# plumk97/pip

Measured on AMD Instinct MI355X. Metric: GiB/s payload checksummed (device-resident), MTU-9000 TCP batch; Mpkt/s, higher is better.
Workload: dtype u8

## Files before the change

### pip_amd/csrc/pipck_coop.hip

```cpp
#include "pipck_common.hpp"
#include "pipck_device.hpp"

#include <algorithm>

namespace pipck {

constexpr uint32_t kCoopLoadsOnly = 1u << 21;
constexpr uint32_t kCoopNoEnd = 1u << 22;

template <int U>
constexpr int coop_waves_per_simd() { return U >= 32 ? 2 : (U >= 24 ? 3 : (U >= 16 ? 4 : 5)); }

__host__ __device__ constexpr uint32_t coop_pitch(uint32_t k) { return k | 1u; }

template <int U, bool VERIFY, bool NT, bool PROBE>
__device__ __forceinline__ void coop_body(uint32_t* s_part, const uint8_t* __restrict__ arena, uint32_t cpp,
                                          uint32_t len, uint64_t n, uint32_t K, const uint32_t* __restrict__ pseudo,
                                          uint32_t n_flows, const uint32_t* __restrict__ flow_of, uint64_t flow_origin,
                                          uint16_t* __restrict__ out, uint8_t* __restrict__ ok, uint32_t kflags,
                                          uint32_t* __restrict__ err) {
    if (!PROBE) kflags &= ~(kCoopLoadsOnly | kCoopNoEnd);
    const int lane = threadIdx.x & 63;
    const uint32_t w = (uint32_t)__builtin_amdgcn_readfirstlane((int)(threadIdx.x >> 6));
    const uint32_t pitch = coop_pitch(K);
    const uint64_t p0 = (uint64_t)blockIdx.x * K;
    const uint32_t np = (uint32_t)min<uint64_t>((uint64_t)K, n - p0);
    const uint32_t tchunks = np * cpp;
    const uint32_t rows = (tchunks + 63) >> 6;
    const uint32_t nch = (len + 15) >> 4;
    const int tail = nch ? (int)len - 16 * ((int)nch - 1) : 16;
    for (uint32_t i = threadIdx.x; i < 64u * pitch; i += 256) s_part[i] = 0;
    uint32_t Pb = 0;
    bool fbad = false;
    if (pseudo && threadIdx.x < np) {
        const uint64_t pkt = p0 + threadIdx.x;
        Pb = flow_of ? flow_pseudo(pseudo, flow_of[pkt], n_flows, fbad)
                     : pseudo[(uint32_t)((flow_origin + pkt) % n_flows)];
    }
    __syncthreads();
    const buf_t tb = buf_rsrc(reinterpret_cast<const u32x4*>(arena) + p0 * cpp, tchunks * 16u);
    uint32_t* part = s_part + lane * pitch;
    const uint32_t q = 256u / cpp, rm = 256u % cpp;
    uint32_t pkt = (64u * w) / cpp, k0 = (64u * w) % cpp;
    const uint32_t my_rows = rows > w ? (rows - w + 3) >> 2 : 0u;
    u32x4 v[U];
    uint32_t probe = 0;
#pragma unroll
    for (int u = 0; u < U; u++) v[u] = buf_load<NT>(tb, ((w + 4u * u) * 64u + lane) * 16u);
    for (uint32_t j0 = 0; j0 < my_rows; j0 += U) {
#pragma unroll
        for (int u = 0; u < U; u++) {
            const uint32_t j = j0 + u;
            if (j < my_rows && (kflags & kCoopLoadsOnly)) {
                probe += v[u].x;
            } else if (j < my_rows) {
                uint32_t k = k0 + lane, pk = pkt;
                if (k >= cpp) {
                    k -= cpp;
                    pk++;
                }
                u32x4 x = v[u];
                if (k >= nch) x = u32x4{0u, 0u, 0u, 0u};
                else if (k == nch - 1 && tail < 16) x = mask_tail(x, tail);
                if (pk < np) atomicAdd(&part[pk], dot4(x, 0u));
                k0 += rm;
                pkt += q;
                if (k0 >= cpp) {
                    k0 -= cpp;
                    pkt++;
                }
            }
            v[u] = buf_load<NT>(tb, ((w + 4u * (j + U)) * 64u + lane) * 16u);
        }
    }
    __syncthreads();
    if (kflags & (kCoopLoadsOnly | kCoopNoEnd)) {
        if (probe == 0x9E3779B9u) s_part[0] = probe;
        return;
    }
    const uint32_t i = threadIdx.x;
    if (i < np) {
        uint32_t s = 0;
#pragma unroll 16
        for (int l = 0; l < 64; l++) s += s_part[l * pitch + i];
        const uint32_t F = bswap16(fold16(s));
        const uint32_t P = pseudo ? Pb + len_term(len) : 0u;
        if (fbad) flow_refused(err);
        if (VERIFY)
            store_result8(buf_rsrc(ok + p0, np), i, fbad ? 0u : (uint32_t)(fold16(P + F) == 0xFFFFu));
        else
            store_result16(buf_rsrc(out + p0, 2u * np), 2u * i, fbad ? 0u : (uint32_t)finish(P, F));
    }
}

template <int U, bool VERIFY, bool NT>
__global__ __launch_bounds__(256) __attribute__((amdgpu_waves_per_eu(coop_waves_per_simd<U>()))) void k_flat_coop(
    const uint8_t* __restrict__ arena, uint32_t cpp, uint32_t len, uint64_t n, uint32_t K,
    const uint32_t* __restrict__ pseudo, uint32_t n_flows, const uint32_t* __restrict__ flow_of, uint64_t flow_origin,
    uint16_t* __restrict__ out, uint8_t* __restrict__ ok, uint32_t kflags, uint32_t* __restrict__ err) {
    extern __shared__ uint32_t s_part[];
    coop_body<U, VERIFY, NT, false>(s_part, arena, cpp, len, n, K, pseudo, n_flows, flow_of, flow_origin, out, ok,
                                    kflags, err);
}

template <int U, bool VERIFY, bool NT>
__global__ __launch_bounds__(256) __attribute__((amdgpu_waves_per_eu(coop_waves_per_simd<U>()))) void
k_flat_coop_probe(const uint8_t* __restrict__ arena, uint32_t cpp, uint32_t len, uint64_t n, uint32_t K,
                  const uint32_t* __restrict__ pseudo, uint32_t n_flows, const uint32_t* __restrict__ flow_of,
                  uint64_t flow_origin, uint16_t* __restrict__ out, uint8_t* __restrict__ ok, uint32_t kflags,
                  uint32_t* __restrict__ err) {
    extern __shared__ uint32_t s_part[];
    coop_body<U, VERIFY, NT, true>(s_part, arena, cpp, len, n, K, pseudo, n_flows, flow_of, flow_origin, out, ok,
                                   kflags, err);
}

typedef void (*coop_fn)(const uint8_t*, uint32_t, uint32_t, uint64_t, uint32_t, const uint32_t*, uint32_t,
                        const uint32_t*, uint64_t, uint16_t*, uint8_t*, uint32_t, uint32_t*);

int launch_flat_coop(bool verify, const void* d_arena, uint64_t stride, uint32_t len, uint64_t n,
                     const uint32_t* d_pseudo, uint32_t n_flows, const uint32_t* d_flow_of, uint64_t flow_origin,
                     uint16_t* d_out, uint8_t* d_ok, uint32_t* d_err, hipStream_t s, uint32_t rows_per_wave,
                     uint32_t ring, uint32_t kflags) {
    const uint32_t cpp = (uint32_t)(stride / 16);
    const bool jumbo = cpp >= 256;
    const uint32_t rpw = rows_per_wave ? rows_per_wave : (jumbo ? 64u : 48u);
    uint32_t K = (4u * rpw * 64u) / cpp;
    K = std::max<uint32_t>(8u, std::min<uint32_t>(256u, K / 8u * 8u));
    if ((uint64_t)K * cpp * 16u >= (1ull << 31)) return PIPCK_EINVAL;
    const uint64_t blocks = (n + K - 1) / K;
    if (blocks > 0x7FFFFFFFull) return PIPCK_EINVAL;
    const size_t lds = 64u * coop_pitch(K) * sizeof(uint32_t);
    const uint32_t nf = n_flows ? n_flows : 1u;
    const uint32_t u = ring ? ring : 32u;
    static const coop_fn kCoop[3][2] = {
        {k_flat_coop<16, false, true>, k_flat_coop<16, true, true>},
        {k_flat_coop<24, false, true>, k_flat_coop<24, true, true>},
        {k_flat_coop<32, false, true>, k_flat_coop<32, true, true>}};
    static const coop_fn kCoopProbe[3] = {k_flat_coop_probe<16, false, true>, k_flat_coop_probe<24, false, true>,
                                          k_flat_coop_probe<32, false, true>};
    const int ui = u >= 32 ? 2 : (u >= 24 ? 1 : 0);
    const bool probe = (kflags & (kCoopLoadsOnly | kCoopNoEnd)) && !verify;
    PIPCK_LAUNCH(probe ? kCoopProbe[ui] : kCoop[ui][verify], dim3((uint32_t)blocks), dim3(256), lds, s, (const uint8_t*)d_arena, cpp, len, n,
                 K, d_pseudo, nf, d_flow_of, flow_origin, d_out, d_ok, kflags, d_err);
    PIPCK_LAUNCHED("k_flat_coop");
    return PIPCK_OK;
}

}
```

### pip_amd/engine.py

```python
from __future__ import annotations

import ctypes as C

from . import _lib
from ._lib import Desc, Flow4, Flow6, call, check, load

DESC_BYTES = C.sizeof(Desc)


def _torch():
    import torch

    return torch


def _ptr(t) -> C.c_void_p | None:
    return None if t is None else C.c_void_p(t.data_ptr())


def current_stream(device=None) -> C.c_void_p:
    torch = _torch()
    return C.c_void_p(torch.cuda.current_stream(device).cuda_stream)


def require_gpu() -> None:
    torch = _torch()
    if not torch.cuda.is_available():
        raise RuntimeError("pip_amd engine needs a HIP device (gfx950); none is visible")
    load()


_hip = None


def hip_runtime() -> C.CDLL:
    global _hip
    if _hip is None:
        import os

        load()
        paths = set()
        with open("/proc/self/maps") as f:
            for line in f:
                parts = line.split()
                if len(parts) >= 6 and os.path.basename(parts[5]).startswith("libamdhip64.so"):
                    paths.add(os.path.realpath(parts[5]))
        if len(paths) != 1:
            raise RuntimeError(f"expected exactly one HIP runtime mapped in this process, found {sorted(paths)}")
        _hip = C.CDLL(paths.pop(), mode=os.RTLD_NOLOAD | os.RTLD_GLOBAL)
    return _hip


def pci_bus_id(device: int) -> str:
    buf = C.create_string_buffer(64)
    try:
        if hip_runtime().hipDeviceGetPCIBusId(buf, C.c_int(len(buf)), C.c_int(device)) == 0:
            return buf.value.decode()
    except (OSError, RuntimeError):
        pass
    p = _torch().cuda.get_device_properties(device)
    return f"{getattr(p, 'pci_domain_id', 0):04x}:{getattr(p, 'pci_bus_id', 0):02x}:" \
           f"{getattr(p, 'pci_device_id', 0):02x}.0"


def gen_flows(family: int, n_flows: int, seed: int, proto: int, device=None):
    torch = _torch()
    size = C.sizeof(Flow4 if family == 4 else Flow6)
    flows = torch.empty(n_flows * size, dtype=torch.uint8, device=device or "cuda")
    fn = "pipck_gen_flows4" if family == 4 else "pipck_gen_flows6"
    call(fn, _ptr(flows), n_flows, seed, proto, current_stream(flows.device))
    return flows, prepare_flows(family, flows, n_flows)


def prepare_flows(family: int, flows, n_flows: int):
    torch = _torch()
    pseudo = torch.empty(n_flows, dtype=torch.int32, device=flows.device)
    fn = "pipck_flows4_prepare" if family == 4 else "pipck_flows6_prepare"
    call(fn, _ptr(flows), n_flows, _ptr(pseudo), current_stream(flows.device))
    return pseudo


def flows_to_device(family: int, flows_bytes: bytes, device=None):
    torch = _torch()
    t = torch.frombuffer(bytearray(flows_bytes), dtype=torch.uint8).to(device or "cuda")
    return t


def _n_flows(n_flows, pseudo, flow_of) -> int:
    if n_flows is not None:
        return n_flows
    if flow_of is not None and pseudo is not None:
        return pseudo.numel()
    return 1


def checksum_fixed(arena, stride: int, length: int, n: int, pseudo=None, n_flows: int | None = None, flow_of=None,
                   flow_origin: int = 0, out=None, err=None):
    torch = _torch()
    if out is None:
        out = torch.empty(n, dtype=torch.int16, device=arena.device)
    _check_span(arena, stride, length, n)
    call("pipck_checksum_fixed_n", _ptr(arena), stride, length, n, _ptr(pseudo), _n_flows(n_flows, pseudo, flow_of),
         _ptr(flow_of), flow_origin, _ptr(out), _ptr(err), current_stream(arena.device))
    return out


def _bound(fn: str, *args):
    f = getattr(load(), fn)

    def run():
        rc = f(*args)
        if rc:
            check(fn, rc)

    return run


def prepare_checksum_fixed(arena, stride: int, length: int, n: int, pseudo=None, n_flows: int | None = None,
                           flow_of=None, flow_origin: int = 0, out=None, err=None):
    torch = _torch()
    if out is None:
        out = torch.empty(n, dtype=torch.int16, device=arena.device)
    _check_span(arena, stride, length, n)
    return _bound("pipck_checksum_fixed_n", _ptr(arena), stride, length, n, _ptr(pseudo),
                  _n_flows(n_flows, pseudo, flow_of), _ptr(flow_of), flow_origin, _ptr(out), _ptr(err),
                  current_stream(arena.device)), out


def verify_fixed(arena, stride: int, length: int, n: int, pseudo=None, n_flows: int | None = None, flow_of=None,
                 flow_origin: int = 0, ok=None, err=None):
    torch = _torch()
    if ok is None:
        ok = torch.empty(n, dtype=torch.uint8, device=arena.device)
    _check_span(arena, stride, length, n)
    call("pipck_verify_fixed_n", _ptr(arena), stride, length, n, _ptr(pseudo), _n_flows(n_flows, pseudo, flow_of),
         _ptr(flow_of), flow_origin, _ptr(ok), _ptr(err), current_stream(arena.device))
    return ok


def checksum_ragged(arena, desc, pseudo=None, out=None, err=None):
    torch = _torch()
    n = desc.shape[0]
    if out is None:
        out = torch.empty(n, dtype=torch.int16, device=arena.device)
    call("pipck_checksum_ragged_n", _ptr(arena), _nbytes(arena), _ptr(desc), n, _ptr(pseudo),
         pseudo.numel() if pseudo is not None else 0, _ptr(out), _ptr(err), current_stream(arena.device))
    return out


def verify_ragged(arena, desc, pseudo=None, ok=None, err=None):
    torch = _torch()
    n = desc.shape[0]
    if ok is None:
        ok = torch.empty(n, dtype=torch.uint8, device=arena.device)
    call("pipck_verify_ragged_n", _ptr(arena), _nbytes(arena), _ptr(desc), n, _ptr(pseudo),
         pseudo.numel() if pseudo is not None else 0, _ptr(ok), _ptr(err), current_stream(arena.device))
    return ok


def tune_xcd_weights(m=None, period: int = 0) -> None:
    arr = (C.c_uint32 * 8)(*[int(x) for x in m]) if m is not None else None
    call("pipck_tune_xcd_weights", arr, period)


def _nbytes(t) -> int:
    return t.numel() * t.element_size()


def checksum_packed(arena, lens, tile_chunk, n: int | None = None, pseudo=None, n_flows: int | None = None,
                    flow_of=None, flow_origin: int = 0, out=None, err=None):
    torch = _torch()
    n = lens.numel() if n is None else n
    if out is None:
        out = torch.empty(n, dtype=torch.int16, device=arena.device)
    _check_packed(arena, lens, tile_chunk, n)
    call("pipck_checksum_packed_n", _ptr(arena), _nbytes(arena), _ptr(lens), _ptr(tile_chunk), n, _ptr(pseudo),
         _n_flows(n_flows, pseudo, flow_of), _ptr(flow_of), flow_origin, _ptr(out), _ptr(err),
         current_stream(arena.device))
    return out


def verify_packed(arena, lens, tile_chunk, n: int | None = None, pseudo=None, n_flows: int | None = None,
                  flow_of=None, flow_origin: int = 0, ok=None, err=None):
    torch = _torch()
    n = lens.numel() if n is None else n
    if ok is None:
        ok = torch.empty(n, dtype=torch.uint8, device=arena.device)
    _check_packed(arena, lens, tile_chunk, n)
    call("pipck_verify_packed_n", _ptr(arena), _nbytes(arena), _ptr(lens), _ptr(tile_chunk), n, _ptr(pseudo),
         _n_flows(n_flows, pseudo, flow_of), _ptr(flow_of), flow_origin, _ptr(ok), _ptr(err),
         current_stream(arena.device))
    return ok


def packed_index(lens, n: int | None = None):
    torch = _torch()
    n = lens.numel() if n is None else n
    tc = torch.empty((n + 63) // 64 + 1, dtype=torch.int64, device=lens.device)
    call("pipck_packed_index", _ptr(lens), n, _ptr(tc), current_stream(lens.device))
    return tc


_packed_total: dict = {}


def _check_packed(arena, lens, tile_chunk, n, unit: int = 16):
    import weakref

    if n > lens.numel() or tile_chunk.numel() < (n + 63) // 64 + 1:
        raise ValueError("lens / tile_chunk shorter than the batch")
    ent = _packed_total.get(id(tile_chunk))
    if ent is not None and ent[0]() is tile_chunk and ent[1] == tile_chunk._version and ent[2] == n:
        chunks = ent[3]
    else:
        chunks = int(tile_chunk[(n + 63) // 64].item())
        if len(_packed_total) > 64:
            _packed_total.clear()
        _packed_total[id(tile_chunk)] = (weakref.ref(tile_chunk), tile_chunk._version, n, chunks)
    need = unit * chunks if unit == 16 else (chunks + 15) // 16 * 16
    if need > arena.numel() * arena.element_size():
        raise ValueError(f"packed batch needs {need} B, arena has {arena.numel() * arena.element_size()}")


def checksum_packed_bytes(arena, lens, tile_off, n: int | None = None, pseudo=None, n_flows: int | None = None,
                          flow_of=None, flow_origin: int = 0, out=None, err=None):
    torch = _torch()
    n = lens.numel() if n is None else n
    if out is None:
        out = torch.empty(n, dtype=torch.int16, device=arena.device)
    _check_packed(arena, lens, tile_off, n, unit=1)
    call("pipck_checksum_packed_bytes_n", _ptr(arena), _nbytes(arena), _ptr(lens), _ptr(tile_off), n, _ptr(pseudo),
         _n_flows(n_flows, pseudo, flow_of), _ptr(flow_of), flow_origin, _ptr(out), _ptr(err),
         current_stream(arena.device))
    return out


def prepare_checksum_packed_bytes(arena, lens, tile_off, n: int | None = None, pseudo=None,
                                  n_flows: int | None = None, flow_of=None, flow_origin: int = 0, out=None, err=None):
    torch = _torch()
    n = lens.numel() if n is None else n
    if out is None:
        out = torch.empty(n, dtype=torch.int16, device=arena.device)
    _check_packed(arena, lens, tile_off, n, unit=1)
    return _bound("pipck_checksum_packed_bytes_n", _ptr(arena), _nbytes(arena), _ptr(lens), _ptr(tile_off), n,
                  _ptr(pseudo), _n_flows(n_flows, pseudo, flow_of), _ptr(flow_of), flow_origin, _ptr(out),
                  _ptr(err), current_stream(arena.device)), out


def verify_packed_bytes(arena, lens, tile_off, n: int | None = None, pseudo=None, n_flows: int | None = None,
                        flow_of=None, flow_origin: int = 0, ok=None, err=None):
    torch = _torch()
    n = lens.numel() if n is None else n
    if ok is None:
        ok = torch.empty(n, dtype=torch.uint8, device=arena.device)
    _check_packed(arena, lens, tile_off, n, unit=1)
    call("pipck_verify_packed_bytes_n", _ptr(arena), _nbytes(arena), _ptr(lens), _ptr(tile_off), n, _ptr(pseudo),
         _n_flows(n_flows, pseudo, flow_of), _ptr(flow_of), flow_origin, _ptr(ok), _ptr(err),
         current_stream(arena.device))
    return ok


def rx_verify_ring(ring, stride: int, lens, n: int | None = None, ok=None, err=None):
    torch = _torch()
    n = lens.numel() if n is None else n
    if n * stride > _nbytes(ring) or n > lens.numel():
        raise ValueError("ring smaller than n * stride, or fewer lengths than slots")
    if ok is None:
        ok = torch.empty(n, dtype=torch.uint8, device=ring.device)
    call("pipck_rx_verify_ring_n", _ptr(ring), stride, _ptr(lens), n, _ptr(ok), _ptr(err),
         current_stream(ring.device))
    return ok


def rx_verify_device(arena, lens, tile_off, n: int | None = None, ok=None, err=None):
    torch = _torch()
    n = lens.numel() if n is None else n
    if ok is None:
        ok = torch.empty(n, dtype=torch.uint8, device=arena.device)
    _check_packed(arena, lens, tile_off, n, unit=1)
    call("pipck_rx_verify_device", _ptr(arena), _nbytes(arena), _ptr(lens), _ptr(tile_off), n, _ptr(ok), _ptr(err),
         current_stream(arena.device))
    return ok


TX_IP_FILLED, TX_L4_FILLED = 1, 2
TX_UDP_ZERO_AS_ONES = 1


def tx_fill_device(arena, lens, tile_off, n: int | None = None, flags: int = 0, done=None, err=None):
    torch = _torch()
    n = lens.numel() if n is None else n
    if done is None:
        done = torch.empty(n, dtype=torch.uint8, device=arena.device)
    _check_packed(arena, lens, tile_off, n, unit=1)
    call("pipck_tx_fill_device", _ptr(arena), _nbytes(arena), _ptr(lens), _ptr(tile_off), n, flags, _ptr(done),
         _ptr(err), current_stream(arena.device))
    return done


def packed_bytes_index(lens, n: int | None = None):
    torch = _torch()
    n = lens.numel() if n is None else n
    to = torch.empty((n + 63) // 64 + 1, dtype=torch.int64, device=lens.device)
    call("pipck_packed_bytes_index", _ptr(lens), n, _ptr(to), current_stream(lens.device))
    return to


def checksum_chains(arena, segs, seg_begin, pkt_flow=None, pseudo=None, out=None, err=None):
    torch = _torch()
    n_pk = seg_begin.shape[0] - 1
    scratch = torch.empty(max(segs.shape[0], 1), dtype=torch.int32, device=arena.device)
    if out is None:
        out = torch.empty(n_pk, dtype=torch.int16, device=arena.device)
    call("pipck_checksum_chains_n", _ptr(arena), _nbytes(arena), _ptr(segs), segs.shape[0], _ptr(seg_begin),
         _ptr(pkt_flow), n_pk, _ptr(pseudo), pseudo.numel() if pseudo is not None else 0, _ptr(scratch), _ptr(out),
         _ptr(err), current_stream(arena.device))
    return out


def update_fixed(arena, stride: int, n: int, cover_off: int, cover_len: int, ck_off: int, edit_off: int,
                 edit_len: int, new_bytes=None, new_stride: int = 0, pseudo_old=None, pseudo_new=None,
                 n_flows: int | None = None, flow_of=None, flow_origin: int = 0, err=None) -> None:
    if pseudo_old is not None and pseudo_new is not None and pseudo_old.numel() != pseudo_new.numel():
        raise ValueError("pseudo_old and pseudo_new must have the same number of flows")
    _check_span(arena, stride, cover_off + cover_len, n)
    if edit_len and new_bytes is not None and n and \
            (n - 1) * new_stride + edit_len > new_bytes.numel() * new_bytes.element_size():
        raise ValueError("new_bytes is too small for the batch")
    call("pipck_update_fixed_n", _ptr(arena), stride, n, cover_off, cover_len, ck_off, edit_off, edit_len,
         _ptr(new_bytes), new_stride, _ptr(pseudo_old), _ptr(pseudo_new), _n_flows(n_flows, pseudo_old, flow_of),
         _ptr(flow_of), flow_origin, _ptr(err), current_stream(arena.device))


def _check_span(arena, stride, length, n):
    if n and (n - 1) * stride + length > arena.numel() * arena.element_size():
        raise ValueError(f"arena of {arena.numel() * arena.element_size()} B is too small for "
                         f"{n} packets x stride {stride} (len {length})")


def make_desc(offsets, lengths, flows, device=None):
    import numpy as np

    torch = _torch()
    n = len(offsets)
    raw = np.zeros(n, dtype=[("offset", "<u8"), ("len", "<u4"), ("flow", "<u4")])
    raw["offset"], raw["len"], raw["flow"] = offsets, lengths, flows
    return torch.from_numpy(raw.view(np.int64).reshape(n, 2).copy()).to(device or "cuda")


def cfg_seed(cfg: int) -> int:
    return load().pipck_cfg_seed(cfg)


def gen_fixed(arena, stride: int, length: int, n: int, first: int, seed: int, hdr: int) -> None:
    _check_span(arena, stride, length, n)
    if n and (n * stride) > arena.numel() * arena.element_size():
        raise ValueError("arena too small for generated stride slots")
    call("pipck_gen_fixed", _ptr(arena), stride, length, n, first, seed, hdr, current_stream(arena.device))


def gen_ragged(n: int, first: int, seed: int, hdr: int, n_flows: int, device=None, lengths=None):
    torch = _torch()
    dev = device or "cuda"
    if lengths is None:
        lengths = torch.empty(n, dtype=torch.int32, device=dev)
        call("pipck_gen_zipf_lengths", _ptr(lengths), n, first, seed, current_stream(lengths.device))
    desc = torch.empty((n, 2), dtype=torch.int64, device=lengths.device)
    nbytes = C.c_uint64(0)
    call("pipck_gen_ragged_layout", _ptr(lengths), n, first, n_flows, _ptr(desc), C.byref(nbytes),
         current_stream(lengths.device))
    arena = torch.empty(max(int(nbytes.value), 16), dtype=torch.uint8, device=lengths.device)
    call("pipck_gen_ragged_fill", _ptr(arena), _ptr(desc), n, first, seed, hdr, current_stream(arena.device))
    return arena, desc, lengths


def gen_packed(n: int, first: int, seed: int, hdr: int, device=None, lengths=None):
    torch = _torch()
    arena, desc, lengths = gen_ragged(n, first, seed, hdr, 1, device=device, lengths=lengths)
    del desc
    lens16 = lengths.to(torch.int16)
    return arena, lens16, packed_index(lens16, n), lengths


def gen_packed_bytes(n: int, first: int, seed: int, hdr: int, device=None, lengths=None):
    torch = _torch()
    dev = device or "cuda"
    if lengths is None:
        lengths = torch.empty(n, dtype=torch.int32, device=dev)
        call("pipck_gen_zipf_lengths", _ptr(lengths), n, first, seed, current_stream(lengths.device))
    lens16 = lengths.to(torch.int16)
    tile_off = packed_bytes_index(lens16, n)
    total = int(tile_off[(n + 63) // 64].item())
    arena = torch.empty(max((total + 15) // 16 * 16, 16), dtype=torch.uint8, device=lengths.device)
    arena[total:].zero_()
    call("pipck_gen_packed_bytes", _ptr(arena), _ptr(lens16), _ptr(tile_off), n, first, seed, hdr,
         current_stream(arena.device))
    return arena, lens16, tile_off, lengths


def gen_rx_ring(n: int, seed: int, stride: int, l4_len: int = 0):
    torch = _torch()
    arena, lens, _, kind, start, l4 = gen_rx_frames(n, seed, l4_len=l4_len)
    ln = lens.to(torch.int64) & 0xFFFF
    if int(ln.max().item()) > stride:
        raise ValueError("a frame is longer than the slot stride")
    ring = torch.zeros(n * stride, dtype=torch.uint8, device=arena.device)
    step = 1 << 16
    for f0 in range(0, n, step):
        lc, sc = ln[f0:f0 + step], start[f0:f0 + step]
        m = lc.numel()
        frame = torch.repeat_interleave(torch.arange(m, device=arena.device), lc)
        excl = torch.cumsum(lc, 0) - lc
        within = torch.arange(frame.numel(), device=arena.device) - excl[frame]
        ring[(f0 + frame) * stride + within] = arena[sc[frame] + within]
    return ring, lens, kind


def gen_rx_frames(n: int, seed: int, checksummed: bool = True, l4_len: int = 0):
    torch = _torch()
    g = torch.Generator(device="cuda").manual_seed(seed)
    l4 = torch.empty(n, dtype=torch.int32, device="cuda")
    if l4_len:
        l4.fill_(l4_len)
    else:
        call("pipck_gen_zipf_lengths", _ptr(l4), n, 0, cfg_seed(4), current_stream())
    kind = torch.randint(0, 4, (n,), device="cuda", generator=g)
    v6 = kind == 3
    hl = torch.where(v6, 40, 20).to(torch.int64)
    l4 = l4.to(torch.int64)
    frame = l4 + hl
    lens = frame.to(torch.int16)
    tile_off = packed_bytes_index(lens)
    total = int(tile_off[-1].item())
    arena = torch.randint(0, 256, ((total + 16 + 127) // 128 * 128,), dtype=torch.uint8, device="cuda", generator=g)
    start = torch.cumsum(frame, 0) - frame
    proto = torch.where(kind == 2, 17, 6)

    def put(col, val, mask):
        idx = (start + col)[mask]
        arena[idx] = (val[mask] if torch.is_tensor(val) else torch.full_like(idx, val)).to(torch.uint8)

    v4 = ~v6
    put(0, 0x45, v4)
    put(2, frame >> 8, v4)
    put(3, frame & 0xFF, v4)
    put(6, 0, v4)
    put(7, 0, v4)
    put(9, proto, v4)
    put(0, 0x60, v6)
    put(4, l4 >> 8, v6)
    put(5, l4 & 0xFF, v6)
    put(6, 6, v6)
    if not checksummed:
        return arena, lens, tile_off, kind, start, l4
    field = start + hl + torch.where(proto == 6, 16, 6)
    for k in (0, 1):
        arena[field + k] = 0
    put(10, 0, v4)
    put(11, 0, v4)

    def be_words(first, count):
        idx = start[:, None] + first + torch.arange(2 * count, device="cuda")
        b = arena[idx].to(torch.int64)
        return (b[:, 0::2] * 256 + b[:, 1::2]).sum(1)

    pseudo = torch.where(v6, be_words(8, 16), be_words(12, 4)) + proto
    flows = torch.arange(n, device="cuda", dtype=torch.int64)

    def ragged(off, ln, ps):
        desc = torch.stack([off, ln | (flows << 32)], 1)
        return checksum_ragged(arena, desc, ps).to(torch.int64) & 0xFFFF

    r = ragged(start + hl, l4, pseudo.to(torch.int32))
    arena[field] = (r >> 8).to(torch.uint8)
    arena[field + 1] = (r & 0xFF).to(torch.uint8)
    ip = ragged(start, torch.full_like(l4, 20), None)
    put(10, ip >> 8, v4)
    put(11, ip & 0xFF, v4)
    return arena, lens, tile_off, kind, start, l4


def tune(lanes_per_packet: int = 0, loads_per_lane: int = 0, blocks: int = 0, plain_loads: bool = False,
         flat: bool = True, nt_loads: bool = False, rows_per_task: int = 0, xcd_groups: bool = False,
         packed_tiles: bool = True, wide_blocks: bool = False,
         small: bool = True, small_k_log: int = 0, flat_small: bool = True, tiny_tiles: bool = True,
         flat_tiny: bool = True, force_flat_tiny: bool = False, packed_marks_only: bool = False,
         trace: bool = False, loads_only: bool = False, no_task_end: bool = False,
         end_no_store: bool = False, alt_flat_schedule: bool = False,
         plain_result_stores: bool = False, wave_stores: bool = False, free_run: bool = False,
         packed_no_align: bool = False, hdr_in_place: bool = False, ring_own_slots: bool = False,
         ring_all_coop: bool = False, ring_adapt: bool | None = None) -> None:
    if not 0 <= small_k_log <= 4:
        raise ValueError("small_k_log must be 0..4")
    flags = ((1 if plain_loads else 0) | (0 if flat else 2) | (4 if nt_loads else 0) | (8 if xcd_groups else 0)
             | (0 if packed_tiles else 16) | (32 if wide_blocks else 0) | (0 if small else 64)
             | (0 if flat_small else 128) | (rows_per_task << 8) | (0 if tiny_tiles else 1 << 16)
             | (0 if flat_tiny else 1 << 17) | (1 << 18 if force_flat_tiny else 0) | (small_k_log << 24)
             | (1 << 19 if packed_marks_only else 0) | (1 << 20 if trace else 0) | (1 << 21 if loads_only else 0) | (1 << 22 if no_task_end else 0)
             | (1 << 23 if end_no_store else 0) | (1 << 28 if alt_flat_schedule else 0)
             | (1 << 29 if plain_result_stores else 0)
             | (1 << 30 if (wave_stores or packed_no_align) else 0)
             | (1 << 31 if free_run else 0))
    load().pipck_tune(lanes_per_packet, loads_per_lane, blocks, flags)
    load().pipck_tune_probes(1 if hdr_in_place else 0)
    ring = (1 if ring_own_slots else 0) | (2 if ring_all_coop else 0) | {None: 0, False: 4, True: 8}[ring_adapt]
    if ring or hasattr(load(), "pipck_tune_ring"):
        load().pipck_tune_ring(ring)
```

Before: 6743.

## Pin coop kernel load pipeline with explicit vmcnt waits and sched barriers

Inserts explicit s_waitcnt vmcnt(U-1) and scheduling barriers around each ring-buffer load so the compiler keeps U outstanding buffer loads in flight, instead of reordering or over-waiting. It also fixes waves_per_eu to an exact min/max per unroll depth and adds U=28/36/56 variants selectable through the ring parameter. An optional LDS padding cap limits coop blocks per CU through a new tune knob. The hand-coded vmcnt encoding and the barriers could block useful compiler scheduling, and the tighter occupancy bound could cause register spills.

```diff
diff --git a/pip_amd/csrc/pipck_coop.hip b/pip_amd/csrc/pipck_coop.hip
--- a/pip_amd/csrc/pipck_coop.hip
+++ b/pip_amd/csrc/pipck_coop.hip
@@ -8,8 +8,17 @@
 constexpr uint32_t kCoopLoadsOnly = 1u << 21;
 constexpr uint32_t kCoopNoEnd = 1u << 22;
 
+
 template <int U>
-constexpr int coop_waves_per_simd() { return U >= 32 ? 2 : (U >= 24 ? 3 : (U >= 16 ? 4 : 5)); }
+constexpr int coop_waves_per_simd() { return U > 36 ? 2 : (U > 28 ? 3 : (U > 16 ? 4 : 6)); }
+
+constexpr int coop_vmcnt(int n) { return (n & 15) | ((n >> 4) << 14) | 0x0F70; }
+
+constexpr uint32_t kLdsPerCu = 160u * 1024u;
+constexpr size_t coop_cap_lds(uint32_t blocks_per_cu) {
+    return blocks_per_cu >= 2 && blocks_per_cu <= 8 ? (size_t)(kLdsPerCu / (blocks_per_cu + 1u) / 2048u + 1u) * 2048u
+                                                    : 0u;
+}
 
 __host__ __device__ constexpr uint32_t coop_pitch(uint32_t k) { return k | 1u; }
 
@@ -46,11 +55,16 @@
     u32x4 v[U];
     uint32_t probe = 0;
 #pragma unroll
-    for (int u = 0; u < U; u++) v[u] = buf_load<NT>(tb, ((w + 4u * u) * 64u + lane) * 16u);
+    for (int u = 0; u < U; u++) {
+        v[u] = buf_load<NT>(tb, ((w + 4u * u) * 64u + lane) * 16u);
+        __builtin_amdgcn_sched_barrier(0);
+    }
     for (uint32_t j0 = 0; j0 < my_rows; j0 += U) {
 #pragma unroll
         for (int u = 0; u < U; u++) {
             const uint32_t j = j0 + u;
+            __builtin_amdgcn_s_waitcnt(coop_vmcnt(U - 1));
+            __builtin_amdgcn_sched_barrier(0);
             if (j < my_rows && (kflags & kCoopLoadsOnly)) {
                 probe += v[u].x;
             } else if (j < my_rows) {
@@ -70,7 +84,9 @@
                     pkt++;
                 }
             }
+            __builtin_amdgcn_sched_barrier(0);
             v[u] = buf_load<NT>(tb, ((w + 4u * (j + U)) * 64u + lane) * 16u);
+            __builtin_amdgcn_sched_barrier(0);
         }
     }
     __syncthreads();
@@ -94,7 +110,8 @@
 }
 
 template <int U, bool VERIFY, bool NT>
-__global__ __launch_bounds__(256) __attribute__((amdgpu_waves_per_eu(coop_waves_per_simd<U>()))) void k_flat_coop(
+__global__ __launch_bounds__(256)
+__attribute__((amdgpu_waves_per_eu(coop_waves_per_simd<U>(), coop_waves_per_simd<U>()))) void k_flat_coop(
     const uint8_t* __restrict__ arena, uint32_t cpp, uint32_t len, uint64_t n, uint32_t K,
     const uint32_t* __restrict__ pseudo, uint32_t n_flows, const uint32_t* __restrict__ flow_of, uint64_t flow_origin,
     uint16_t* __restrict__ out, uint8_t* __restrict__ ok, uint32_t kflags, uint32_t* __restrict__ err) {
@@ -104,7 +121,8 @@
 }
 
 template <int U, bool VERIFY, bool NT>
-__global__ __launch_bounds__(256) __attribute__((amdgpu_waves_per_eu(coop_waves_per_simd<U>()))) void
+__global__ __launch_bounds__(256)
+__attribute__((amdgpu_waves_per_eu(coop_waves_per_simd<U>(), coop_waves_per_simd<U>()))) void
 k_flat_coop_probe(const uint8_t* __restrict__ arena, uint32_t cpp, uint32_t len, uint64_t n, uint32_t K,
                   const uint32_t* __restrict__ pseudo, uint32_t n_flows, const uint32_t* __restrict__ flow_of,
                   uint64_t flow_origin, uint16_t* __restrict__ out, uint8_t* __restrict__ ok, uint32_t kflags,
@@ -129,16 +147,18 @@
     if ((uint64_t)K * cpp * 16u >= (1ull << 31)) return PIPCK_EINVAL;
     const uint64_t blocks = (n + K - 1) / K;
     if (blocks > 0x7FFFFFFFull) return PIPCK_EINVAL;
-    const size_t lds = 64u * coop_pitch(K) * sizeof(uint32_t);
+    const uint32_t cap = (ring >> 8) & 0xFu;
+    const size_t lds = std::max<size_t>(64u * coop_pitch(K) * sizeof(uint32_t), coop_cap_lds(cap));
     const uint32_t nf = n_flows ? n_flows : 1u;
-    const uint32_t u = ring ? ring : 32u;
-    static const coop_fn kCoop[3][2] = {
-        {k_flat_coop<16, false, true>, k_flat_coop<16, true, true>},
-        {k_flat_coop<24, false, true>, k_flat_coop<24, true, true>},
-        {k_flat_coop<32, false, true>, k_flat_coop<32, true, true>}};
-    static const coop_fn kCoopProbe[3] = {k_flat_coop_probe<16, false, true>, k_flat_coop_probe<24, false, true>,
-                                          k_flat_coop_probe<32, false, true>};
-    const int ui = u >= 32 ? 2 : (u >= 24 ? 1 : 0);
+    const uint32_t u = (ring & 0xFFu) ? (ring & 0xFFu) : 32u;
+#define PIPCK_COOP_U(U) {k_flat_coop<U, false, true>, k_flat_coop<U, true, true>}
+    static const coop_fn kCoop[6][2] = {
+        PIPCK_COOP_U(16), PIPCK_COOP_U(24), PIPCK_COOP_U(28), PIPCK_COOP_U(32), PIPCK_COOP_U(36), PIPCK_COOP_U(56)};
+#undef PIPCK_COOP_U
+    static const coop_fn kCoopProbe[6] = {k_flat_coop_probe<16, false, true>, k_flat_coop_probe<24, false, true>,
+                                          k_flat_coop_probe<28, false, true>, k_flat_coop_probe<32, false, true>,
+                                          k_flat_coop_probe<36, false, true>, k_flat_coop_probe<56, false, true>};
+    const int ui = u >= 56 ? 5 : (u >= 36 ? 4 : (u >= 32 ? 3 : (u >= 28 ? 2 : (u >= 24 ? 1 : 0))));
     const bool probe = (kflags & (kCoopLoadsOnly | kCoopNoEnd)) && !verify;
     PIPCK_LAUNCH(probe ? kCoopProbe[ui] : kCoop[ui][verify], dim3((uint32_t)blocks), dim3(256), lds, s, (const uint8_t*)d_arena, cpp, len, n,
                  K, d_pseudo, nf, d_flow_of, flow_origin, d_out, d_ok, kflags, d_err);
diff --git a/pip_amd/engine.py b/pip_amd/engine.py
--- a/pip_amd/engine.py
+++ b/pip_amd/engine.py
@@ -489,7 +489,10 @@
          end_no_store: bool = False, alt_flat_schedule: bool = False,
          plain_result_stores: bool = False, wave_stores: bool = False, free_run: bool = False,
          packed_no_align: bool = False, hdr_in_place: bool = False, ring_own_slots: bool = False,
-         ring_all_coop: bool = False, ring_adapt: bool | None = None) -> None:
+         ring_all_coop: bool = False, ring_adapt: bool | None = None, coop_blocks_per_cu: int = 0) -> None:
+    if coop_blocks_per_cu and not 2 <= coop_blocks_per_cu <= 8:
+        raise ValueError("coop_blocks_per_cu must be 0 or 2..8")
+    loads_per_lane |= coop_blocks_per_cu << 8
     if not 0 <= small_k_log <= 4:
         raise ValueError("small_k_log must be 0..4")
     flags = ((1 if plain_loads else 0) | (0 if flat else 2) | (4 if nt_loads else 0) | (8 if xcd_groups else 0)
```

Result: no change. 6750, median of 6 (+0.1%).
